# ultravideo/uvg266

Measured on AMD Instinct MI355X. Metric: encoded fps (1080p all-intra --preset medium closed loop: CTU search with the reference's RD decisions -> deblock -> SAO -> slice data; Mpixels/s in config), higher is better.
Workload: dtype u8

## Files before the change

### uvg266_amd/csrc/ctu_core.h

```cpp
#pragma once
#include <stdint.h>
#include <stddef.h>
#include <string.h>
#include "intra_pred_dev.h"
#if defined(__HIPCC__)
#include "satd_dev.h"
#endif
#include "vvc_tables.h"
#include "vvc_ctx_init.h"
#include "vvc_rdoq_tables.h"
#include "../../include/uvg266_hip.h"
#if defined(CTU_PB)
#include "inter_cand_dev.h"
#endif

#if defined(__HIPCC__)
#define CTU_NOINLINE __attribute__((noinline))
#define CTU_INLINE __attribute__((always_inline))
#define CTU_INLINE1 __attribute__((always_inline))
#define CTU_DEV static __device__
#define CTU_SHARED __shared__
#define CTU_TID ((int)(threadIdx.x & 63))
#define CTU_NT 64
#define CTU_WAVE (__builtin_amdgcn_readfirstlane((int)((threadIdx.x >> 6) - S->rot) & 3))
#define CTU_SYNC() do { __builtin_amdgcn_fence(__ATOMIC_ACQ_REL, "wavefront"); __builtin_amdgcn_wave_barrier(); } while (0)
#define BLK_TID ((int)threadIdx.x)
#define BLK_NT ((int)blockDim.x)
#define BLK_SYNC() __syncthreads()
#define CTU_GLOAD(p) __builtin_nontemporal_load(p)
#define CTU_LDS __attribute__((address_space(3)))
#define CTU_GLB __attribute__((address_space(1)))
#else
#define CTU_NOINLINE
#define CTU_INLINE
#define CTU_INLINE1
#define CTU_DEV static inline
#define CTU_SHARED static
#define CTU_TID 0
#define CTU_NT 1
#define CTU_WAVE (ctu::g_emul_wave)
#define CTU_SYNC() ((void)0)
#define BLK_TID 0
#define BLK_NT 1
#define BLK_SYNC() ((void)0)
#define CTU_GLOAD(p) (*(p))
#define CTU_LDS
#define CTU_GLB
#endif
#if defined(CTU_PB)
#define CTU_RQ_ROOT(V) ((V)->rq_root)
#else
#define CTU_RQ_ROOT(V) 0
#endif
#if defined(__HIPCC__) && defined(CTU_PROFILE)
#define CTU_T0() const unsigned long long ctu_t0__ = __builtin_amdgcn_s_memtime()
#define CTU_T1(W, slot) do { if (CTU_TID == 0) (W)->prof[CTU_WAVE][slot] += __builtin_amdgcn_s_memtime() - ctu_t0__; } while (0)
#define RQ_T0(W) scratch *const rq_w__ = (W); unsigned long long tq = __builtin_amdgcn_s_memtime();
#define RQ_T(slot) do { const unsigned long long t2 = __builtin_amdgcn_s_memtime(); if (CTU_TID == 0) rq_w__->prof[CTU_WAVE][slot] += t2 - tq; tq = t2; } while (0)
#define LF_T0() unsigned long long tq = __builtin_amdgcn_s_memtime()
#define LF_T(slot) do { const unsigned long long t2 = __builtin_amdgcn_s_memtime(); if (CTU_TID == 0 && CTU_WAVE == 0) J.W->prof_lf[slot] += t2 - tq; tq = t2; } while (0)
#define LF_TR() do { tq = __builtin_amdgcn_s_memtime(); } while (0)
#define LF_TN(slot) do { const unsigned long long t2 = __builtin_amdgcn_s_memtime(); if (CTU_TID == 0 && CTU_WAVE == 0) J.W->prof_lf[slot] += (1ull << 40) + (t2 - tq); tq = t2; } while (0)
#define WAIT_EVAL(S, L) do { LF_T0(); wait_eval(S, L); LF_T((L) <= 2 ? 14 : 15); } while (0)
#define CTU_PROF_RESET(S, J) BLK_FOR(i, 4 * 32) (J).W->prof[i >> 5][i & 31] = 0; BLK_FOR(i, 16) (J).W->prof_lf[i] = 0; (S)->prof_w = (J).W;
#define PB_T0() const unsigned long long pb_t0__ = __builtin_amdgcn_s_memtime()
#if defined(CTU_PROFILE_WALK)
#define PB_T1(W, slot) do { if (CTU_TID == 0 && ((slot) >= 14 || CTU_WAVE == 0)) (W)->prof_pb[slot] += __builtin_amdgcn_s_memtime() - pb_t0__; } while (0)
#else
#define PB_T1(W, slot) do { if (CTU_TID == 0) (W)->prof_pb[slot] += __builtin_amdgcn_s_memtime() - pb_t0__; } while (0)
#endif
#define PB_COUNT(W, slot) SERIAL (W)->prof_pb[slot] += 1;
#define PB_PROF_RESET(S, J) BLK_FOR(i, 24) (J).W->prof_pb[i] = 0; BLK_FOR(i, 4 * 32) (J).W->prof[i >> 5][i & 31] = 0; (S)->prof_w = (J).W;
#else
#define CTU_T0() ((void)0)
#define CTU_T1(W, slot) ((void)0)
#define RQ_T0(W)
#define RQ_T(slot) ((void)0)
#define LF_T0() ((void)0)
#define LF_T(slot) ((void)0)
#define LF_TR() ((void)0)
#define LF_TN(slot) ((void)0)
#define WAIT_EVAL(S, L) wait_eval(S, L)
#define CTU_PROF_RESET(S, J)
#define PB_T0() ((void)0)
#define PB_T1(W, slot) ((void)0)
#define PB_COUNT(W, slot)
#define PB_PROF_RESET(S, J)
#endif
#define LDSP(T, p) ((CTU_LDS T *)(p))
#define MGP(PX, T, p) ((typename ctu::mg_ptr<PX, T>::type)(p))
#define PAR_FOR(i, n) for (int i = CTU_TID; i < (n); i += CTU_NT)
#define BLK_FOR(i, n) for (int i = BLK_TID; i < (n); i += BLK_NT)
#define SERIAL if (CTU_TID == 0)

namespace ctu {

#if !defined(__HIPCC__)
static int g_emul_wave = 0;
static int g_emul_lazy = 0;
static int g_emul_depthwave = 0;
static int g_emul_leafwave = 0;
template <typename F> static inline void emul_on_wave(int w, F fn)
{
  const int me = g_emul_wave;
  g_emul_wave = w;
  fn();
  g_emul_wave = me;
}
#endif

enum { LCU = 64, LCU_C = 32, PY = 68, PC = 36, NMODELS = 257 };
#if defined(CTU_PB)
enum { NMX = NMODELS + 18 };
#else
enum { NMX = NMODELS };
#endif
enum { M_SIGGRP = 0, M_SIG = 4, M_PAR = 28, M_GT1 = 70, M_GT2 = 112, M_LASTX = 154, M_LASTY = 194, M_CBF_LUMA = 234, M_CBF_CB = 238,
       M_CBF_CR = 240, M_SPLIT = 244, M_MPM = 253, M_PLANAR = 254, M_CHROMA_PRED = 256 };
enum { CU_NOTSET = 0, CU_INTRA = 1, CU_INTER = 2 };
#define CTU_MAX_DOUBLE 1.7976931348623157e308

using params = uvghip_ctu_params_t;

struct cu4 {
  uint8_t type, log2, cbf, luma_edges, chroma_edges, log2_c;
  int8_t mode, mode_chroma;
};

struct level_state {
  double cost, split_cost, split_bits;
  int x, y;
  int child;
  int type, mode, cbf;
  int has_chroma;
  int pending;
  int evalp, known, can;
  uint32_t split_tree, mode_type_tree;
#if defined(CTU_PB)
  int32_t mot[8];
  uint8_t fl[8];
  int32_t cbf4[4];
#endif
};

#if !defined(__HIPCC__)
template <typename PX> struct lds_cfg { enum { slim = 0, slim_scan = 0 }; };
#elif defined(CTU_PB)
template <typename PX> struct lds_cfg { enum { slim = 0, slim_scan = 1 }; };
#else
template <typename PX> struct lds_cfg { enum { slim = 0, slim_scan = 0 }; };
template <> struct lds_cfg<uint16_t> { enum { slim = 1, slim_scan = 1 }; };
#endif
template <typename PX, typename T, bool SLIM = (lds_cfg<PX>::slim != 0)> struct mg_ptr { typedef CTU_LDS T *type; };
template <typename PX, typename T> struct mg_ptr<PX, T, true> { typedef T *type; };

template <typename PX> struct px_info;
template <> struct px_info<uint8_t> { enum { depth = 8, maxv = 255 }; };
template <> struct px_info<uint16_t> { enum { depth = 10, maxv = 1023 }; };

struct wctx {
// ... 158 lines not shown
template <typename PX> struct job {
  params P;
  const PX *src_y, *src_u, *src_v;
  int src_stride, src_stride_c;
  PX *rec_y, *rec_u, *rec_v;
  int rec_stride, rec_stride_c;
  uvghip_scu_t *cu_tab;
  int cu_stride;
  int16_t *coeff;
  uint32_t *models_out;
  const uint32_t *models_in;
  scratch *W;
  int x, y;
#if defined(CTU_PB)
  const struct pb_job *pb;
  uint32_t *pbm_out;
  const uint32_t *pbm_in;
  int slice_type, init_qp;
#endif
};

template <typename PX> CTU_DEV CTU_GLB const PX *src_block(const job<PX> &J, int color, int bx, int by, int *pitch)
{
  const PX *p = color == 0 ? J.src_y : (color == 1 ? J.src_u : J.src_v);
  const int st = color == 0 ? J.src_stride : J.src_stride_c, sh = color != 0;
  *pitch = st;
  return (CTU_GLB const PX *)(p + (size_t)((J.y >> sh) + by) * st + (J.x >> sh) + bx);
}


CTU_DEV uint32_t *tab_ebits() { CTU_SHARED uint32_t t[512]; return t; }
CTU_DEV uint8_t *tab_rate() { CTU_SHARED uint8_t t[(NMX + 7) & ~7]; return t; }
CTU_DEV uint32_t *tab_rdoq_bits() { CTU_SHARED uint32_t t[2 * 244]; return t; }
#define kRate (tab_rate())

template <typename MP> CTU_DEV int m_state(MP m, int c) { return (int)(((m[c] & 0xffffu) + (m[c] >> 16)) >> 8); }
template <typename MP> CTU_DEV void m_update(MP m, int c, int bin)
{
  const int r0 = kRate[c] >> 4, r1 = kRate[c] & 15;
  uint32_t s0 = m[c] & 0xffffu, s1 = m[c] >> 16;
  s0 -= (s0 >> r0) & 0x7fe0u;
  s1 -= (s1 >> r1) & 0x7ffeu;
  if (bin) { s0 += (0x7fffu >> r0) & 0x7fe0u; s1 += (0x7fffu >> r1) & 0x7ffeu; }
  m[c] = (s0 & 0xffffu) | (s1 << 16);
}
template <typename MP> CTU_DEV double m_fbits(MP m, int c, int bin) { return (double)tab_ebits()[(m_state(m, c) << 1) ^ bin] / 32768.0; }
template <typename MP> CTU_DEV void m_code(MP m, int update, int c, int bin, double &bits)
{
  bits += m_fbits(m, c, bin);
  if (update) m_update(m, c, bin);
}

CTU_DEV void models_init_one(uint32_t *m, int i, int qp, int slice)
{
  const int v = k_ctx_init[slice][i];
  if (v == 255) { m[i] = 0; return; }
  const int slope = (v >> 3) - 4, offset = ((v & 7) * 18) + 1;
  int s = ((slope * (qp - 16)) >> 1) + offset;
  s = s < 1 ? 1 : (s > 127 ? 127 : s);
  const uint32_t p1 = (uint32_t)s << 8;
  m[i] = (p1 & 0x7fe0u) | ((p1 & 0x7ffeu) << 16);
}

CTU_DEV int scan_base(int log2n) { return log2n == 5 ? 0 : log2n == 4 ? 1024 : log2n == 3 ? 1280 : 1344; }
template <typename PX> CTU_DEV uint16_t *scan_of(lds<PX> *S, int log2n)
{
  if (lds_cfg<PX>::slim_scan) return log2n >= 4 ? S->scr->scan_g + (log2n == 5 ? 0 : 1024) : S->scan + (log2n == 3 ? 0 : 64);
  return S->scan + scan_base(log2n);
}
CTU_DEV int last_bits_off(int t, int log2n, int xy)
{
  const int cnt = 2 * log2n;
  const int base = log2n == 2 ? 0 : (log2n == 3 ? 8 : (log2n == 4 ? 20 : 36));
  return (t ? 56 : 0) + base + (xy ? cnt : 0);
}
CTU_DEV void diag_order(int n, uint8_t *out)
{
  int i = 0;
  for (int d = 0; d < 2 * n - 1; ++d)
    for (int x = 0; x <= d; ++x) {
      const int y = d - x;
      if (x < n && y < n) out[i++] = (uint8_t)(y * n + x);
    }
}
template <typename PX> CTU_DEV void build_scans(lds<PX> *S)
{
  SERIAL {
    uint8_t in[16], cg[64];
    diag_order(4, in);
    for (int l2 = 2; l2 <= 5; ++l2) {
      const int n = 1 << l2, cgw = n >> 2;
      diag_order(cgw, cg);
      uint16_t *sc = scan_of(S, l2);
      if (l2 == 2) {
        for (int k = 0; k < 16; ++k) S->inv4[in[k]] = (uint8_t)k;
        for (int k = 0; k < 16; ++k) {
          const int x = in[k] & 3, y = in[k] >> 2;
          unsigned m = 0;
          if (x + 1 < 4) m |= 1u << S->inv4[y * 4 + x + 1];
          if (x + 2 < 4) m |= 1u << S->inv4[y * 4 + x + 2];
          if (y + 1 < 4) m |= 1u << S->inv4[(y + 1) * 4 + x];
          if (y + 2 < 4) m |= 1u << S->inv4[(y + 2) * 4 + x];
          if (x + 1 < 4 && y + 1 < 4) m |= 1u << S->inv4[(y + 1) * 4 + x + 1];
          S->deps4[k] = (uint16_t)m;
        }
      }
      for (int g = 0; g < cgw * cgw; ++g) {
        const int gx = cg[g] % cgw, gy = cg[g] / cgw;
        for (int k = 0; k < 16; ++k) sc[g * 16 + k] = (uint16_t)((gy * 4 + in[k] / 4) * n + gx * 4 + in[k] % 4);
      }
    }
  }
  CTU_SYNC();
}

CTU_DEV int16_t *lv_of(wctx *V, int color) { return color == 0 ? V->lv0 : (color == 1 ? V->lv1 : V->lv2); }
template <typename PX> CTU_DEV PX *plane(lds<PX> *S, int color) { return color == 0 ? S->Dy : (color == 1 ? S->Du : S->Dv); }
CTU_DEV int pitch_of(int color) { return color == 0 ? PY : PC; }
template <typename PX> CTU_DEV cu4 *cu_at(lds<PX> *S, int lx, int ly) { return &S->cu[((ly >> 2) + 1) * 17 + (lx >> 2) + 1]; }

template <typename PX> CTU_DEV int count_edge_cus(lds<PX> *S, int x, int y, int lx, int ly, int n, int left)
{
  if ((left && x == 0) || (!left && y == 0)) return 0;
  if (left && lx == 0) return (LCU - ly) / 4;
  if (!left && ly == 0) return n / 2;
  int amount = n & ~3;
  if (left) {
    if (ly == 0 && lx == 32 && cu_at(S, lx, ly)->log2 == 6) return 8;
    while (ly + amount < LCU && cu_at(S, lx - 4, ly + amount)->type != CU_NOTSET) amount += 4;
  } else {
    while (lx + amount < LCU && cu_at(S, lx + amount, ly - 4)->type != CU_NOTSET) amount += 4;
  }
  return (amount / 4) > (n / 4) ? amount / 4 : n / 4;
}

template <typename PX> CTU_NOINLINE CTU_DEV void build_refs(lds<PX> *S, const params &P, int color, int x, int y, int lx, int ly, int n, int cu_n)
{
  wctx *const V = wv_of(S);
  const int c = color != 0;
  const int w = n >> c;
  const int px_x = lx >> c, px_y = ly >> c;
  const int pit = pitch_of(color);
  const PX *D = plane(S, color) + (px_y + 1) * pit + px_x + 1;
  SERIAL {
    int al = count_edge_cus(S, x, y, lx, ly, n, 1) * (c ? 2 : 4);
    if (al > 2 * w) al = 2 * w;
    if (al > ((P.pic_h - y) >> c)) al = (P.pic_h - y) >> c;
    int at = count_edge_cus(S, x, y, lx, ly, n, 0) * (c ? 2 : 4);
    if (at > 2 * w) at = 2 * w;
    if (at > ((P.pic_w - x) >> c)) at = (P.pic_w - x) >> c;
    if (x > 0 && y > 0 && P.wpp && px_y == 0 && at > (LCU >> c) - px_x) at = (LCU >> c) - px_x;
    V->u_avail_left = al; V->u_avail_top = at;
  }
  CTU_SYNC();
  const int al = V->u_avail_left, at = V->u_avail_top;
  const int dc = 1 << (px_info<PX>::depth - 1);
  CTU_LDS uint16_t *const r_top = LDSP(uint16_t, V->top), *const r_left = LDSP(uint16_t, V->left);
  CTU_LDS uint16_t *const r_ftop = LDSP(uint16_t, V->ftop), *const r_fleft = LDSP(uint16_t, V->fleft);
  PAR_FOR(i, V->refn - 1) {
    int lv, tv;
    if (x > 0) lv = D[(i < al ? i : al - 1) * pit - 1];
    else lv = y > 0 ? D[-pit] : dc;
    if (y > 0) tv = D[-pit + (i < at ? i : at - 1)];
    else tv = x > 0 ? D[-1] : dc;
    r_left[i + 1] = (uint16_t)lv;
    r_top[i + 1] = (uint16_t)tv;
// ... 780 lines not shown
      const int o = off + (ctx >> sh);
      const int mx = M_LASTX + (E.t ? 20 : 0) + o, my = M_LASTY + (E.t ? 20 : 0) + o;
      last_x_bits[ctx] = bx + rbits(E, mx, 0); bx += rbits(E, mx, 1);
      last_y_bits[ctx] = by + rbits(E, my, 0); by += rbits(E, my, 1);
    }
    last_x_bits[ctx] = bx; last_y_bits[ctx] = by;
  }
  int found_last = 0;
  for (cgs = cg_last_scanpos; cgs >= 0; cgs--) {
    const int first = scan[cgs * 16];
    const int cg_blkpos = ((first >> l2) >> 2) * cgw + ((first & (n - 1)) >> 2);
    base_cost -= cost_cg_sig[cgs];
    if (cg_flag[cg_blkpos]) {
      for (int sp = 15; sp >= 0; sp--) {
        const int scanpos = cgs * 16 + sp;
        if (scanpos > last_scanpos) continue;
        const int blkpos = scan[scanpos];
        if (dst[blkpos]) {
          const int pos_y = blkpos >> l2, pos_x = blkpos - (pos_y << l2);
          const int cx = group_idx(pos_x), cy = group_idx(pos_y);
          double cl = last_x_bits[cx] + last_y_bits[cy];
          if (cx > 3) cl += 32768 * ((cx - 2) >> 1);
          if (cy > 3) cl += 32768 * ((cy - 2) >> 1);
          const double cost_last = lambda * cl;
          const double total = base_cost + cost_last - cost_sig[scanpos];
          if (total < best_cost) { best_last_idx_p1 = scanpos + 1; best_cost = total; }
          if (dst[blkpos] > 1) { found_last = 1; break; }
          base_cost -= cost_coeff[scanpos];
          base_cost += cost_coeff0[scanpos];
        } else {
          base_cost -= cost_sig[scanpos];
        }
      }
      if (found_last) break;
    }
  }
  int any = 0;
  for (int scanpos = 0; scanpos < best_last_idx_p1; scanpos++) {
    const int b = scan[scanpos], level = dst[b];
    any |= level;
    dst[b] = (int16_t)((coef[b] < 0) ? -level : level);
  }
  for (int scanpos = best_last_idx_p1; scanpos <= last_scanpos; scanpos++) dst[scan[scanpos]] = 0;
  return any != 0;
}

struct rdoq_pos { int level; double cc, cs; };
template <typename DP> CTU_INLINE CTU_DEV rdoq_pos rdoq_decide_inl(const rdoq_env &E, CTU_LDS const int16_t *coef, DP dst, int n, int l2, int color, int blkpos, bool is_last,
                             bool regular, int go_rice, double c0, int *mal_out)
{
  const int cap_half = 1 << (E.q_bits - 1);
  const int64_t prod = (int64_t)iabs_((int)coef[blkpos]) * E.q;
  const int32_t cap = 0x7fffffff - cap_half;
  const int32_t level_double = (int32_t)(prod < cap ? prod : cap);
  const uint32_t max_abs_level = (uint32_t)(level_double + cap_half) >> E.q_bits;
  const int pos_y = blkpos >> l2, pos_x = blkpos - (pos_y << l2);
  int ctx_sig = 0, ctx_set = 0;
  if (!is_last) {
    int diag, tsum;
    ctx_sig = sig_ctx_abs(dst, pos_x, pos_y, n, color, &diag, &tsum);
    ctx_set = ((tsum < 4 ? tsum : 4) + 1) + (!diag ? ((color == 0) ? 15 : 5) : (color == 0) ? (diag < 3 ? 10 : (diag < 10 ? 5 : 0)) : 0);
  }
  if (!regular) go_rice = go_rice_par(template_abs_sum(dst, 0, pos_x, pos_y, n));
  rdoq_pos r;
  r.cs = 0;
  r.level = (int)coded_level(E, &r.cc, c0, &r.cs, level_double, max_abs_level, ctx_sig, ctx_set, go_rice, regular ? 4u : 0u, is_last);
  *mal_out = (int)max_abs_level;
  return r;
}
template <typename DP> CTU_NOINLINE CTU_DEV rdoq_pos rdoq_decide(const rdoq_env &E, CTU_LDS const int16_t *coef, DP dst, int n, int l2, int color, int blkpos, bool is_last,
                             bool regular, int go_rice, double c0, int *mal_out)
{
  return rdoq_decide_inl(E, coef, dst, n, l2, color, blkpos, is_last, regular, go_rice, c0, mal_out);
}

#if !defined(__HIPCC__)
#include "ctu_rdoq_emul.h"
#else
CTU_DEV double rl64(double v, int lane)
{
  const int lo = __builtin_amdgcn_readlane(__double2loint(v), lane), hi = __builtin_amdgcn_readlane(__double2hiint(v), lane);
  return __hiloint2double(hi, lo);
}
template <typename PX> CTU_INLINE1 CTU_DEV void rdoq_wave(lds<PX> *S, scratch *W, const int16_t *coef_, int16_t *dst_, int n, int color, int cbf_u, int qp_scaled,
                                              double lambda, int bitdepth)
{
  wctx *const V = wv_of(S);
  CTU_LDS const int16_t *const coef = LDSP(const int16_t, coef_);
  typename mg_ptr<PX, int16_t>::type const dst = MGP(PX, int16_t, dst_);
  const int l2 = ilog2_dev(n), nn = n * n, cgw = n >> 2;
  const uint16_t *scan = scan_of(S, l2);
  rdoq_env E;
  E.st = S->rdoq_state; E.t = color ? 1 : 0; E.lambda = lambda;
  const int transform_shift = 15 - bitdepth - l2;
  E.q_bits = 14 + qp_scaled / 6 + transform_shift;
  E.q = kQuantScales[qp_scaled % 6];
  double scale = 32768;
  scale = transform_shift >= 0 ? scale / kPow2[2 * transform_shift] : scale * kPow2[-2 * transform_shift];
  E.error_scale = scale / E.q / E.q;
  const bool small = V->rq_cc != nullptr;
  CTU_LDS double *const CCl = LDSP(double, V->rq_cc), *const CSl = LDSP(double, V->rq_cs);
  const bool d1 = S->vsel[CTU_WAVE] == 3;
  double *const CCg = d1 ? W->cost_coeff : W->cost_coeff0, *const CSg = d1 ? W->cost_sig : W->cost_coeff0 + 512;
  double *cost_cg_sig = (double *)V->t1;
  const int cap_half = 1 << (E.q_bits - 1);
  const int32_t cap = 0x7fffffff - cap_half;
  RQ_T0(W)
  int my_last = -1;
  PAR_FOR(sp, nn) {
    const int blk = scan[sp];
    const int64_t prod = (int64_t)iabs_((int)coef[blk]) * E.q;
    const int32_t level_double = (int32_t)(prod < cap ? prod : cap);
    const int mal = (int)((uint32_t)(level_double + cap_half) >> E.q_bits);
    dst[blk] = (int16_t)mal;
    if (mal > 0 && sp > my_last) my_last = sp;
    if (sp < 64) V->cg_flag[sp] = 0;
  }
  for (int o = 32; o >= 1; o >>= 1) { const int v = __shfl_xor(my_last, o, 64); my_last = v > my_last ? v : my_last; }
  const int last_scanpos = my_last;
  CTU_SYNC();
  if (last_scanpos < 0) { if (CTU_TID == 0) V->rq_i[1] = 0; CTU_SYNC(); return; }
  RQ_T(12);
  const int cg_last = last_scanpos >> 4;
  const int lane = CTU_TID, sp = lane & 15;
  const bool own = lane < 16;
  double tail_cost = 0;
  {
    const auto tail_c0 = [&](int top) -> double {
      const int scanpos = top + sp;
      const int64_t prod = (int64_t)iabs_((int)coef[scan[scanpos]]) * E.q;
      const double err = (double)(int32_t)(prod < cap ? prod : cap);
      return scanpos > last_scanpos ? err * err * E.error_scale : 0.0;
    };
    double nxt = nn - 1 > last_scanpos ? tail_c0(nn - 16) : 0.0;
    for (int top = nn - 16; top + 15 > last_scanpos; top -= 16) {
      const double c0 = nxt;
      if (top - 1 > last_scanpos) nxt = tail_c0(top - 16);
#pragma unroll
      for (int k = 15; k >= 8; --k) tail_cost += rl64(c0, k);
      if (top + 7 > last_scanpos) {
#pragma unroll
        for (int k = 7; k >= 0; --k) tail_cost += rl64(c0, k);
      }
    }
  }
  double block_uncoded_cost = tail_cost, base_cost = tail_cost;
  if (CTU_TID == 0) for (int g = 0; g <= cg_last; ++g) cost_cg_sig[g] = 0;
  int reg_bins = (int)((uint32_t)(nn * 28) >> 4);
  CTU_SYNC();
  RQ_T(13);
  double f_cc = 0, f_cs = 0, f_c0 = 0;
  int f_lev = 0;
  for (int cgs = cg_last; cgs >= 0; --cgs) {
    const int first = scan[cgs * 16];
    const int cg_pos_x = (first & (n - 1)) >> 2, cg_pos_y = (first >> l2) >> 2;
    const int cg_blkpos = cg_pos_y * cgw + cg_pos_x;
    const int regular = reg_bins >= 4;
    const int scanpos = cgs * 16 + sp;
    const bool mine = own && scanpos <= last_scanpos;
    const int blk = scan[mine ? scanpos : cgs * 16];
    const bool is_last = scanpos == last_scanpos;
    const int64_t prod = (int64_t)iabs_((int)coef[blk]) * E.q;
    const int32_t level_double = (int32_t)(prod < cap ? prod : cap);
    const int mal0 = mine ? (int)((uint32_t)(level_double + cap_half) >> E.q_bits) : 0;
    const double c0 = mine ? (double)level_double * (double)level_double * E.error_scale : 0.0;
    int fast = !regular;
    if (regular) {
      int bound = mine ? (mal0 < 2 ? mal0 : 3) + (is_last ? 0 : 1) : 0;
      for (int o = 8; o >= 1; o >>= 1) bound += __shfl_xor(bound, o, 64);
      bound = __builtin_amdgcn_readfirstlane(bound);
      fast = reg_bins - bound >= 4;
    }
    double cc = 0, cs = 0;
    int lev = 0;
    if (fast) {
      int go_rice = 0;
      if (mine && regular && sp != 15 && !is_last) {
        const int nb = scan[scanpos + 1];
        go_rice = go_rice_par(template_abs_sum(coef, 4, nb & (n - 1), nb >> l2, n));
      }
      lev = mal0;
      for (;;) {
        bool changed = false;
        if (mine) {
          int mal;
          const rdoq_pos r = rdoq_decide_inl(E, coef, dst, n, l2, color, blk, is_last, regular != 0, go_rice, c0, &mal);
          cc = r.cc; cs = r.cs;
          changed = r.level != lev;
          lev = r.level;
        }
        CTU_SYNC();
        if (changed) dst[blk] = (int16_t)lev;
        const bool any = __ballot(changed) != 0;
        CTU_SYNC();
        if (!any) break;
      }
    } else {
      if (CTU_TID == 0) {
        int go_rice = 0, rb = reg_bins;
        for (int k = 15; k >= 0; --k) {
          const int spos = cgs * 16 + k;
          if (spos > last_scanpos) continue;
          const int b = scan[spos];
          const int64_t pr = (int64_t)iabs_((int)coef[b]) * E.q;
          const double e0 = (double)(int32_t)(pr < cap ? pr : cap);
          int mal;
          const rdoq_pos r = rdoq_decide(E, coef, dst, n, l2, color, b, spos == last_scanpos, rb >= 4, go_rice, e0 * e0 * E.error_scale, &mal);
          dst[b] = (int16_t)r.level;
          V->rq_stage[k] = r.cc; V->rq_stage[16 + k] = r.cs;
          if ((spos % 16 == 0) && spos > 0) go_rice = 0;
          else if (rb >= 4) {
            rb -= (r.level < 2 ? r.level : 3) + (spos != last_scanpos);
            go_rice = go_rice_par(template_abs_sum(coef, 4, b & (n - 1), b >> l2, n));
          }
        }
        V->rq_i[4] = rb;
      }
      CTU_SYNC();
      if (mine) { cc = V->rq_stage[sp]; cs = V->rq_stage[16 + sp]; lev = dst[blk]; }
      reg_bins = V->rq_i[4];
      CTU_SYNC();
    }
    RQ_T(14);
    double rd_coded = 0, rd_uncoded = 0, rd_sig = 0;
    const unsigned m_nz = (unsigned)__ballot(lev != 0), m_gt1 = (unsigned)__ballot(lev > 1), m_mine = (unsigned)__ballot(mine);
    const unsigned paying = cgs ? ~1u : ~0u, not_last = cgs == cg_last ? ~(1u << (last_scanpos & 15)) : ~0u;
    const int spent = __popc(m_nz & paying) + 2 * __popc(m_gt1 & paying) + __popc(m_mine & paying & not_last);
    const int nnz_before_pos0 = __popc(m_nz & ~1u);
    int flag = cgs && m_nz;
    const bool upper = cgs < cg_last || (last_scanpos & 15) >= 8;
    if (cgs) {
      const double dc = lev ? cc - cs : 0.0, du = lev ? c0 : 0.0;
      if (upper) {
#pragma unroll
        for (int k = 15; k >= 8; --k) {
          block_uncoded_cost += rl64(c0, k); base_cost += rl64(cc, k);
          rd_sig += rl64(cs, k); rd_coded += rl64(dc, k); rd_uncoded += rl64(du, k);
        }
      }
#pragma unroll
      for (int k = 7; k >= 0; --k) {
        block_uncoded_cost += rl64(c0, k); base_cost += rl64(cc, k);
        rd_sig += rl64(cs, k); rd_coded += rl64(dc, k); rd_uncoded += rl64(du, k);
      }
    } else {
      if (upper) {
#pragma unroll
        for (int k = 15; k >= 8; --k) { block_uncoded_cost += rl64(c0, k); base_cost += rl64(cc, k); }
      }
#pragma unroll
      for (int k = 7; k >= 0; --k) { block_uncoded_cost += rl64(c0, k); base_cost += rl64(cc, k); }
    }
    const double rd_sig0 = rl64(cs, 0);
    if (fast && regular) reg_bins -= spent;
    int zeroed = 0;
    if (cgs) {
      unsigned right = 0, lower = 0;
      if (cg_pos_x + 1 < cgw) right = V->cg_flag[cg_blkpos + 1];
      if (cg_pos_y + 1 < cgw) lower = V->cg_flag[cg_blkpos + cgw];
      const int o_grp = M_SIGGRP + (E.t ? 2 : 0) + ((right || lower) ? 1 : 0);
      double cgc = 0;
      if (!flag) {
        cgc = lambda * rbits(E, o_grp, 0);
        base_cost += cgc - rd_sig;
      } else if (cgs < cg_last) {
        if (nnz_before_pos0 == 0) { base_cost -= rd_sig0; rd_sig -= rd_sig0; }
        double cost_zero_cg = base_cost;
        cgc = lambda * rbits(E, o_grp, 1);
        base_cost += cgc;
        cost_zero_cg += lambda * rbits(E, o_grp, 0);
        cost_zero_cg += rd_uncoded;
        cost_zero_cg -= rd_coded;
        cost_zero_cg -= rd_sig;
        if (cost_zero_cg < base_cost) {
          flag = 0;
          zeroed = 1;
          base_cost = cost_zero_cg;
          cgc = lambda * rbits(E, o_grp, 0);
        }
      }
      CTU_SYNC();
      if (CTU_TID == 0) cost_cg_sig[cgs] = cgc;
    } else {
      flag = 1;
    }
    if (CTU_TID == 0) V->cg_flag[cg_blkpos] = (uint8_t)flag;
    if (cg_last == 0) { f_cc = cc; f_cs = cs; f_c0 = c0; f_lev = lev; }
    else if (mine) {
      const double wc = (zeroed && lev) ? c0 : cc, ws = (zeroed && lev) ? 0.0 : cs;
      if (zeroed && lev) dst[blk] = 0;
      if (small) { CCl[scanpos] = wc; CSl[scanpos] = ws; } else { CCg[scanpos] = wc; CSg[scanpos] = ws; }
    }
    CTU_SYNC();
    RQ_T(15);
  }
  RQ_T(16);
  double best_cost;
  int best_last_idx_p1 = 0;
  {
    const int o_cbf = color == 0 ? (CTU_RQ_ROOT(V) ? 243 : M_CBF_LUMA) : color == 1 ? M_CBF_CB : M_CBF_CR + (cbf_u ? 1 : 0);
    best_cost = block_uncoded_cost + lambda * rbits(E, o_cbf, 0);
    base_cost += lambda * rbits(E, o_cbf, 1);
  }
  const int32_t *last_x_bits = S->last_bits + last_bits_off(E.t, l2, 0), *last_y_bits = S->last_bits + last_bits_off(E.t, l2, 1);
  int found_last = 0;
  for (int cgs = cg_last; cgs >= 0 && !found_last; cgs--) {
    const int first = scan[cgs * 16];
    const int cg_blkpos = ((first >> l2) >> 2) * cgw + ((first & (n - 1)) >> 2);
    base_cost -= cost_cg_sig[cgs];
    if (!V->cg_flag[cg_blkpos]) continue;
    const int scanpos = cgs * 16 + sp;
    const bool mine = own && scanpos <= last_scanpos;
    const int blkpos = scan[mine ? scanpos : cgs * 16];
    const int lev = cg_last == 0 ? f_lev : (mine ? (int)dst[blkpos] : 0);
    double kcs = 0, kcc = 0, k0 = 0, klast = 0;
    if (mine) {
      kcs = cg_last == 0 ? f_cs : (small ? CSl[scanpos] : CTU_GLOAD(&CSg[scanpos]));
      if (lev) {
        if (cg_last == 0) { kcc = f_cc; k0 = f_c0; }
        else {
          kcc = small ? CCl[scanpos] : CTU_GLOAD(&CCg[scanpos]);
          const int64_t prod = (int64_t)iabs_((int)coef[blkpos]) * E.q;
          const double err = (double)(int32_t)(prod < cap ? prod : cap);
          k0 = err * err * E.error_scale;
        }
        const int pos_y = blkpos >> l2, pos_x = blkpos - (pos_y << l2);
        const int cx = group_idx(pos_x), cy = group_idx(pos_y);
        double cl = last_x_bits[cx] + last_y_bits[cy];
        if (cx > 3) cl += 32768 * ((cx - 2) >> 1);
        if (cy > 3) cl += 32768 * ((cy - 2) >> 1);
        klast = lambda * cl;
      }
    }
    const double kx = lev ? kcc : kcs;
    const unsigned m_nz = (unsigned)__ballot(lev != 0), m_gt1 = (unsigned)__ballot(lev > 1);
    const int kstop = m_gt1 ? 31 - __clz(m_gt1) : 0;
    const unsigned cand = m_nz >> kstop << kstop;
    if (cgs < cg_last || (last_scanpos & 15) >= 8) {
#pragma unroll
      for (int k = 15; k >= 8; --k) {
        const double total = base_cost + rl64(klast, k) - rl64(kcs, k);
        const bool better = (cand >> k & 1u) != 0 && total < best_cost;
        best_last_idx_p1 = better ? cgs * 16 + k + 1 : best_last_idx_p1;
        best_cost = better ? total : best_cost;
        base_cost = base_cost - rl64(kx, k) + rl64(k0, k);
      }
    }
    if (kstop < 8) {
#pragma unroll
      for (int k = 7; k >= 0; --k) {
        const double total = base_cost + rl64(klast, k) - rl64(kcs, k);
        const bool better = (cand >> k & 1u) != 0 && total < best_cost;
        best_last_idx_p1 = better ? cgs * 16 + k + 1 : best_last_idx_p1;
        best_cost = better ? total : best_cost;
        base_cost = base_cost - rl64(kx, k) + rl64(k0, k);
      }
    }
    found_last = m_gt1 != 0;
  }
  if (CTU_TID == 0) V->rq_i[1] = best_last_idx_p1 > 0;
  RQ_T(17);
  PAR_FOR(scanpos, last_scanpos + 1) {
    const int b = scan[scanpos];
    if (scanpos < best_last_idx_p1) { const int level = dst[b]; dst[b] = (int16_t)((coef[b] < 0) ? -level : level); }
    else dst[b] = 0;
  }
  CTU_SYNC();
  RQ_T(18);
}
#endif

CTU_DEV int coeff_remain_bits(uint32_t remainder, uint32_t rice, unsigned cutoff)
{
  const unsigned threshold = cutoff << rice;
  if (remainder < threshold) return (int)((remainder >> rice) + 1 + rice);
  const unsigned max_prefix = 32 - cutoff - 15;
  unsigned prefix = 0, suffix_len;
  const unsigned code_value = (remainder >> rice) - cutoff;
  if ((int32_t)code_value >= ((1 << max_prefix) - 1)) { prefix = max_prefix; suffix_len = 15; }
  else { while ((int32_t)code_value > ((2 << prefix) - 2)) prefix++; suffix_len = prefix + rice + 1; }
  return (int)(prefix + cutoff + suffix_len);
}
template <typename LP> CTU_DEV int abs_sum_tmpl(LP coeff, int px, int py, int n, int baselevel)
{
  const auto d = coeff + px + py * n;
  int sum = 0;
  if (px < n - 1) {
    sum += iabs_((int)d[1]);
    if (px < n - 2) sum += iabs_((int)d[2]);
    if (py < n - 1) sum += iabs_((int)d[n + 1]);
  }
  if (py < n - 1) {
    sum += iabs_((int)d[n]);
    if (py < n - 2) sum += iabs_((int)d[n << 1]);
  }
  int v = sum - 5 * baselevel;
  v = v < 31 ? v : 31;
  return v > 0 ? v : 0;
}

CTU_NOINLINE CTU_DEV double coeff_bits_serial(uint32_t *m, const uint16_t *scan, const int16_t *coeff, int n, int color)
{
  const int l2 = ilog2_dev(n);
  const int t = color ? 1 : 0;
  const int cgw = n >> 2;
  uint8_t sig_cg[64];
  for (int i = 0; i < cgw * cgw; ++i) sig_cg[i] = 0;
  int scan_pos_last = -1;
  for (int i = 0; i < n * n; ++i)
    if (coeff[scan[i]]) {
      scan_pos_last = i;
      const int f = scan[i & ~15];
      sig_cg[((f >> l2) >> 2) * cgw + ((f & (n - 1)) >> 2)] = 1;
    }
  if (scan_pos_last < 0) return 0;
  const int scan_cg_last = scan_pos_last >> 4;
  double bits_out = 0;
  {
// ... 1684 lines not shown
```

Before: 229.3.

## Batch RDOQ coefficient-group decisions across anti-diagonal using all 64 lanes

```diff
diff --git a/uvg266_amd/csrc/ctu_core.h b/uvg266_amd/csrc/ctu_core.h
--- a/uvg266_amd/csrc/ctu_core.h
+++ b/uvg266_amd/csrc/ctu_core.h
@@ -57,6 +57,7 @@
 #define CTU_T1(W, slot) do { if (CTU_TID == 0) (W)->prof[CTU_WAVE][slot] += __builtin_amdgcn_s_memtime() - ctu_t0__; } while (0)
 #define RQ_T0(W) scratch *const rq_w__ = (W); unsigned long long tq = __builtin_amdgcn_s_memtime();
 #define RQ_T(slot) do { const unsigned long long t2 = __builtin_amdgcn_s_memtime(); if (CTU_TID == 0) rq_w__->prof[CTU_WAVE][slot] += t2 - tq; tq = t2; } while (0)
+#define RQ_N(slot, v) if (CTU_TID == 0) rq_w__->prof[CTU_WAVE][slot] += (unsigned long long)(v) << 40;
 #define LF_T0() unsigned long long tq = __builtin_amdgcn_s_memtime()
 #define LF_T(slot) do { const unsigned long long t2 = __builtin_amdgcn_s_memtime(); if (CTU_TID == 0 && CTU_WAVE == 0) J.W->prof_lf[slot] += t2 - tq; tq = t2; } while (0)
 #define LF_TR() do { tq = __builtin_amdgcn_s_memtime(); } while (0)
@@ -76,6 +77,7 @@
 #define CTU_T1(W, slot) ((void)0)
 #define RQ_T0(W)
 #define RQ_T(slot) ((void)0)
+#define RQ_N(slot, v)
 #define LF_T0() ((void)0)
 #define LF_T(slot) ((void)0)
 #define LF_TR() ((void)0)
@@ -400,6 +402,10 @@
       const int y = d - x;
       if (x < n && y < n) out[i++] = (uint8_t)(y * n + x);
     }
+}
+CTU_DEV int rdoq_diag_start(int n, int d)
+{
+  return d < n ? d * (d + 1) / 2 : n * n - (2 * n - 1 - d) * (2 * n - d) / 2;
 }
 template <typename PX> CTU_DEV void build_scans(lds<PX> *S)
 {
@@ -1346,6 +1352,11 @@
   const int lo = __builtin_amdgcn_readlane(__double2loint(v), lane), hi = __builtin_amdgcn_readlane(__double2hiint(v), lane);
   return __hiloint2double(hi, lo);
 }
+CTU_DEV double shfl64(double v, int from)
+{
+  const int lo = __shfl(__double2loint(v), from, 64), hi = __shfl(__double2hiint(v), from, 64);
+  return __hiloint2double(hi, lo);
+}
 template <typename PX> CTU_INLINE1 CTU_DEV void rdoq_wave(lds<PX> *S, scratch *W, const int16_t *coef_, int16_t *dst_, int n, int color, int cbf_u, int qp_scaled,
                                               double lambda, int bitdepth)
 {
@@ -1413,149 +1424,172 @@
   int reg_bins = (int)((uint32_t)(nn * 28) >> 4);
   CTU_SYNC();
   RQ_T(13);
-  double f_cc = 0, f_cs = 0, f_c0 = 0;
-  int f_lev = 0;
-  for (int cgs = cg_last; cgs >= 0; --cgs) {
-    const int first = scan[cgs * 16];
-    const int cg_pos_x = (first & (n - 1)) >> 2, cg_pos_y = (first >> l2) >> 2;
-    const int cg_blkpos = cg_pos_y * cgw + cg_pos_x;
-    const int regular = reg_bins >= 4;
-    const int scanpos = cgs * 16 + sp;
-    const bool mine = own && scanpos <= last_scanpos;
-    const int blk = scan[mine ? scanpos : cgs * 16];
-    const bool is_last = scanpos == last_scanpos;
-    const int64_t prod = (int64_t)iabs_((int)coef[blk]) * E.q;
-    const int32_t level_double = (int32_t)(prod < cap ? prod : cap);
-    const int mal0 = mine ? (int)((uint32_t)(level_double + cap_half) >> E.q_bits) : 0;
-    const double c0 = mine ? (double)level_double * (double)level_double * E.error_scale : 0.0;
-    int fast = !regular;
-    if (regular) {
-      int bound = mine ? (mal0 < 2 ? mal0 : 3) + (is_last ? 0 : 1) : 0;
-      for (int o = 8; o >= 1; o >>= 1) bound += __shfl_xor(bound, o, 64);
-      bound = __builtin_amdgcn_readfirstlane(bound);
-      fast = reg_bins - bound >= 4;
-    }
-    double cc = 0, cs = 0;
-    int lev = 0;
-    if (fast) {
-      int go_rice = 0;
-      if (mine && regular && sp != 15 && !is_last) {
-        const int nb = scan[scanpos + 1];
-        go_rice = go_rice_par(template_abs_sum(coef, 4, nb & (n - 1), nb >> l2, n));
-      }
-      lev = mal0;
-      for (;;) {
-        bool changed = false;
-        if (mine) {
-          int mal;
-          const rdoq_pos r = rdoq_decide_inl(E, coef, dst, n, l2, color, blk, is_last, regular != 0, go_rice, c0, &mal);
-          cc = r.cc; cs = r.cs;
-          changed = r.level != lev;
-          lev = r.level;
+  const int row = lane >> 4;
+  double cc = 0, cs = 0, c0 = 0;
+  int lev = 0, ng = 0, r = 0, counted = 0;
+  for (int cgs = cg_last; cgs >= 0; --cgs, ++r) {
+    if (r == ng) {
+      const int top = cgs;
+      const int ftop = scan[top * 16];
+      const int dg = ((ftop & (n - 1)) >> 2) + ((ftop >> l2) >> 2);
+      const int dstart = rdoq_diag_start(cgw, dg);
+      ng = top - dstart + 1 < 4 ? top - dstart + 1 : 4;
+      r = 0;
+      const int regular = reg_bins >= 4;
+      const int cgr = row < ng ? top - row : top;
+      const int scanpos = cgr * 16 + sp;
+      const bool mine0 = row < ng && scanpos <= last_scanpos;
+      const int blk = scan[mine0 ? scanpos : cgr * 16];
+      const bool is_last = scanpos == last_scanpos;
+      const int64_t prod = (int64_t)iabs_((int)coef[blk]) * E.q;
+      const int32_t level_double = (int32_t)(prod < cap ? prod : cap);
+      const int mal1 = (int)((uint32_t)(level_double + cap_half) >> E.q_bits);
+      int fast = !regular;
+      if (regular) {
+        int bound = mine0 ? (mal1 < 2 ? mal1 : 3) + (is_last ? 0 : 1) : 0;
+        for (int o = 8; o >= 1; o >>= 1) bound += __shfl_xor(bound, o, 64);
+        const int b0 = __builtin_amdgcn_readlane(bound, 0);
+        const int all = b0 + __builtin_amdgcn_readlane(bound, 16) + __builtin_amdgcn_readlane(bound, 32) + __builtin_amdgcn_readlane(bound, 48);
+        fast = reg_bins - all >= 4;
+        if (!fast && ng > 1) { ng = 1; fast = reg_bins - b0 >= 4; RQ_N(13, 1) }
+      }
+      RQ_N(14, 1) RQ_N(15, ng)
+      const bool mine = mine0 && row < ng;
+      const int mal0 = mine ? mal1 : 0;
+      c0 = mine ? (double)level_double * (double)level_double * E.error_scale : 0.0;
+      cc = 0; cs = 0;
+      lev = 0;
+      counted = fast && regular;
+      if (fast) {
+        int go_rice = 0;
+        if (mine && regular && sp != 15 && !is_last) {
+          const int nb = scan[scanpos + 1];
+          go_rice = go_rice_par(template_abs_sum(coef, 4, nb & (n - 1), nb >> l2, n));
+        }
+        lev = mal0;
+        for (;;) {
+          bool changed = false;
+          RQ_N(12, 1)
+          if (mine) {
+            int mal;
+            const rdoq_pos r = rdoq_decide_inl(E, coef, dst, n, l2, color, blk, is_last, regular != 0, go_rice, c0, &mal);
+            cc = r.cc; cs = r.cs;
+            changed = r.level != lev;
+            lev = r.level;
+          }
+          CTU_SYNC();
+          if (changed) dst[blk] = (int16_t)lev;
+          const bool any = __ballot(changed) != 0;
+          CTU_SYNC();
+          if (!any) break;
+        }
+      } else {
+        if (CTU_TID == 0) {
+          int go_rice = 0, rb = reg_bins;
+          for (int k = 15; k >= 0; --k) {
+            const int spos = top * 16 + k;
+            if (spos > last_scanpos) continue;
+            const int b = scan[spos];
+            const int64_t pr = (int64_t)iabs_((int)coef[b]) * E.q;
+            const double e0 = (double)(int32_t)(pr < cap ? pr : cap);
+            int mal;
+            const rdoq_pos r = rdoq_decide(E, coef, dst, n, l2, color, b, spos == last_scanpos, rb >= 4, go_rice, e0 * e0 * E.error_scale, &mal);
+            dst[b] = (int16_t)r.level;
+            V->rq_stage[k] = r.cc; V->rq_stage[16 + k] = r.cs;
+            if ((spos % 16 == 0) && spos > 0) go_rice = 0;
+            else if (rb >= 4) {
+              rb -= (r.level < 2 ? r.level : 3) + (spos != last_scanpos);
+              go_rice = go_rice_par(template_abs_sum(coef, 4, b & (n - 1), b >> l2, n));
+            }
+          }
+          V->rq_i[4] = rb;
         }
         CTU_SYNC();
-        if (changed) dst[blk] = (int16_t)lev;
-        const bool any = __ballot(changed) != 0;
+        if (mine) { cc = V->rq_stage[sp]; cs = V->rq_stage[16 + sp]; lev = dst[blk]; }
+        reg_bins = V->rq_i[4];
         CTU_SYNC();
-        if (!any) break;
-      }
+      }
+      RQ_T(14);
     } else {
-      if (CTU_TID == 0) {
-        int go_rice = 0, rb = reg_bins;
-        for (int k = 15; k >= 0; --k) {
-          const int spos = cgs * 16 + k;
-          if (spos > last_scanpos) continue;
-          const int b = scan[spos];
-          const int64_t pr = (int64_t)iabs_((int)coef[b]) * E.q;
-          const double e0 = (double)(int32_t)(pr < cap ? pr : cap);
-          int mal;
-          const rdoq_pos r = rdoq_decide(E, coef, dst, n, l2, color, b, spos == last_scanpos, rb >= 4, go_rice, e0 * e0 * E.error_scale, &mal);
-          dst[b] = (int16_t)r.level;
-          V->rq_stage[k] = r.cc; V->rq_stage[16 + k] = r.cs;
-          if ((spos % 16 == 0) && spos > 0) go_rice = 0;
-          else if (rb >= 4) {
-            rb -= (r.level < 2 ? r.level : 3) + (spos != last_scanpos);
-            go_rice = go_rice_par(template_abs_sum(coef, 4, b & (n - 1), b >> l2, n));
+      const int from = (lane + 16) & 63;
+      cc = shfl64(cc, from); cs = shfl64(cs, from); c0 = shfl64(c0, from); lev = __shfl(lev, from, 64);
+    }
+    {
+      const int first = scan[cgs * 16];
+      const int cg_pos_x = (first & (n - 1)) >> 2, cg_pos_y = (first >> l2) >> 2;
+      const int cg_blkpos = cg_pos_y * cgw + cg_pos_x;
+      const int gpos = cgs * 16 + sp;
+      const bool gmine = own && gpos <= last_scanpos;
+      double rd_coded = 0, rd_uncoded = 0, rd_sig = 0;
+      const unsigned m_nz = (unsigned)__ballot(lev != 0) & 0xffffu, m_gt1 = (unsigned)__ballot(lev > 1) & 0xffffu, m_mine = (unsigned)__ballot(gmine);
+      const unsigned paying = cgs ? ~1u : ~0u, not_last = cgs == cg_last ? ~(1u << (last_scanpos & 15)) : ~0u;
+      const int spent = __popc(m_nz & paying) + 2 * __popc(m_gt1 & paying) + __popc(m_mine & paying & not_last);
+      const int nnz_before_pos0 = __popc(m_nz & ~1u);
+      int flag = cgs && m_nz;
+      const bool upper = cgs < cg_last || (last_scanpos & 15) >= 8;
+      if (cgs) {
+        const double dc = lev ? cc - cs : 0.0, du = lev ? c0 : 0.0;
+        if (upper) {
+#pragma unroll
+          for (int k = 15; k >= 8; --k) {
+            block_uncoded_cost += rl64(c0, k); base_cost += rl64(cc, k);
+            rd_sig += rl64(cs, k); rd_coded += rl64(dc, k); rd_uncoded += rl64(du, k);
           }
         }
-        V->rq_i[4] = rb;
-      }
-      CTU_SYNC();
-      if (mine) { cc = V->rq_stage[sp]; cs = V->rq_stage[16 + sp]; lev = dst[blk]; }
-      reg_bins = V->rq_i[4];
-      CTU_SYNC();
-    }
-    RQ_T(14);
-    double rd_coded = 0, rd_uncoded = 0, rd_sig = 0;
-    const unsigned m_nz = (unsigned)__ballot(lev != 0), m_gt1 = (unsigned)__ballot(lev > 1), m_mine = (unsigned)__ballot(mine);
-    const unsigned paying = cgs ? ~1u : ~0u, not_last = cgs == cg_last ? ~(1u << (last_scanpos & 15)) : ~0u;
-    const int spent = __popc(m_nz & paying) + 2 * __popc(m_gt1 & paying) + __popc(m_mine & paying & not_last);
-    const int nnz_before_pos0 = __popc(m_nz & ~1u);
-    int flag = cgs && m_nz;
-    const bool upper = cgs < cg_last || (last_scanpos & 15) >= 8;
-    if (cgs) {
-      const double dc = lev ? cc - cs : 0.0, du = lev ? c0 : 0.0;
-      if (upper) {
 #pragma unroll
-        for (int k = 15; k >= 8; --k) {
+        for (int k = 7; k >= 0; --k) {
           block_uncoded_cost += rl64(c0, k); base_cost += rl64(cc, k);
           rd_sig += rl64(cs, k); rd_coded += rl64(dc, k); rd_uncoded += rl64(du, k);
         }
-      }
+      } else {
+        if (upper) {
 #pragma unroll
-      for (int k = 7; k >= 0; --k) {
-        block_uncoded_cost += rl64(c0, k); base_cost += rl64(cc, k);
-        rd_sig += rl64(cs, k); rd_coded += rl64(dc, k); rd_uncoded += rl64(du, k);
-      }
-    } else {
-      if (upper) {
+          for (int k = 15; k >= 8; --k) { block_uncoded_cost += rl64(c0, k); base_cost += rl64(cc, k); }
+        }
 #pragma unroll
-        for (int k = 15; k >= 8; --k) { block_uncoded_cost += rl64(c0, k); base_cost += rl64(cc, k); }
-      }
-#pragma unroll
-      for (int k = 7; k >= 0; --k) { block_uncoded_cost += rl64(c0, k); base_cost += rl64(cc, k); }
-    }
-    const double rd_sig0 = rl64(cs, 0);
-    if (fast && regular) reg_bins -= spent;
-    int zeroed = 0;
-    if (cgs) {
-      unsigned right = 0, lower = 0;
-      if (cg_pos_x + 1 < cgw) right = V->cg_flag[cg_blkpos + 1];
-      if (cg_pos_y + 1 < cgw) lower = V->cg_flag[cg_blkpos + cgw];
-      const int o_grp = M_SIGGRP + (E.t ? 2 : 0) + ((right || lower) ? 1 : 0);
-      double cgc = 0;
-      if (!flag) {
-        cgc = lambda * rbits(E, o_grp, 0);
-        base_cost += cgc - rd_sig;
-      } else if (cgs < cg_last) {
-        if (nnz_before_pos0 == 0) { base_cost -= rd_sig0; rd_sig -= rd_sig0; }
-        double cost_zero_cg = base_cost;
-        cgc = lambda * rbits(E, o_grp, 1);
-        base_cost += cgc;
-        cost_zero_cg += lambda * rbits(E, o_grp, 0);
-        cost_zero_cg += rd_uncoded;
-        cost_zero_cg -= rd_coded;
-        cost_zero_cg -= rd_sig;
-        if (cost_zero_cg < base_cost) {
-          flag = 0;
-          zeroed = 1;
-          base_cost = cost_zero_cg;
+        for (int k = 7; k >= 0; --k) { block_uncoded_cost += rl64(c0, k); base_cost += rl64(cc, k); }
+      }
+      const double rd_sig0 = rl64(cs, 0);
+      if (counted) reg_bins -= spent;
+      int zeroed = 0;
+      if (cgs) {
+        unsigned right = 0, lower = 0;
+        if (cg_pos_x + 1 < cgw) right = V->cg_flag[cg_blkpos + 1];
+        if (cg_pos_y + 1 < cgw) lower = V->cg_flag[cg_blkpos + cgw];
+        const int o_grp = M_SIGGRP + (E.t ? 2 : 0) + ((right || lower) ? 1 : 0);
+        double cgc = 0;
+        if (!flag) {
           cgc = lambda * rbits(E, o_grp, 0);
+          base_cost += cgc - rd_sig;
+        } else if (cgs < cg_last) {
+          if (nnz_before_pos0 == 0) { base_cost -= rd_sig0; rd_sig -= rd_sig0; }
+          double cost_zero_cg = base_cost;
+          cgc = lambda * rbits(E, o_grp, 1);
+          base_cost += cgc;
+          cost_zero_cg += lambda * rbits(E, o_grp, 0);
+          cost_zero_cg += rd_uncoded;
+          cost_zero_cg -= rd_coded;
+          cost_zero_cg -= rd_sig;
+          if (cost_zero_cg < base_cost) {
+            flag = 0;
+            zeroed = 1;
+            base_cost = cost_zero_cg;
+            cgc = lambda * rbits(E, o_grp, 0);
+          }
         }
+        CTU_SYNC();
+        if (CTU_TID == 0) cost_cg_sig[cgs] = cgc;
+      } else {
+        flag = 1;
+      }
+      if (CTU_TID == 0) V->cg_flag[cg_blkpos] = (uint8_t)flag;
+      if (cg_last != 0 && gmine) {
+        const double wc = (zeroed && lev) ? c0 : cc, ws = (zeroed && lev) ? 0.0 : cs;
+        if (zeroed && lev) dst[scan[gpos]] = 0;
+        if (small) { CCl[gpos] = wc; CSl[gpos] = ws; } else { CCg[gpos] = wc; CSg[gpos] = ws; }
       }
       CTU_SYNC();
-      if (CTU_TID == 0) cost_cg_sig[cgs] = cgc;
-    } else {
-      flag = 1;
-    }
-    if (CTU_TID == 0) V->cg_flag[cg_blkpos] = (uint8_t)flag;
-    if (cg_last == 0) { f_cc = cc; f_cs = cs; f_c0 = c0; f_lev = lev; }
-    else if (mine) {
-      const double wc = (zeroed && lev) ? c0 : cc, ws = (zeroed && lev) ? 0.0 : cs;
-      if (zeroed && lev) dst[blk] = 0;
-      if (small) { CCl[scanpos] = wc; CSl[scanpos] = ws; } else { CCg[scanpos] = wc; CSg[scanpos] = ws; }
-    }
-    CTU_SYNC();
+    }
     RQ_T(15);
   }
   RQ_T(16);
@@ -1576,12 +1610,12 @@
     const int scanpos = cgs * 16 + sp;
     const bool mine = own && scanpos <= last_scanpos;
     const int blkpos = scan[mine ? scanpos : cgs * 16];
-    const int lev = cg_last == 0 ? f_lev : (mine ? (int)dst[blkpos] : 0);
+    const int klev = cg_last == 0 ? lev : (mine ? (int)dst[blkpos] : 0);
     double kcs = 0, kcc = 0, k0 = 0, klast = 0;
     if (mine) {
-      kcs = cg_last == 0 ? f_cs : (small ? CSl[scanpos] : CTU_GLOAD(&CSg[scanpos]));
-      if (lev) {
-        if (cg_last == 0) { kcc = f_cc; k0 = f_c0; }
+      kcs = cg_last == 0 ? cs : (small ? CSl[scanpos] : CTU_GLOAD(&CSg[scanpos]));
+      if (klev) {
+        if (cg_last == 0) { kcc = cc; k0 = c0; }
         else {
           kcc = small ? CCl[scanpos] : CTU_GLOAD(&CCg[scanpos]);
           const int64_t prod = (int64_t)iabs_((int)coef[blkpos]) * E.q;
@@ -1596,8 +1630,8 @@
         klast = lambda * cl;
       }
     }
-    const double kx = lev ? kcc : kcs;
-    const unsigned m_nz = (unsigned)__ballot(lev != 0), m_gt1 = (unsigned)__ballot(lev > 1);
+    const double kx = klev ? kcc : kcs;
+    const unsigned m_nz = (unsigned)__ballot(klev != 0), m_gt1 = (unsigned)__ballot(klev > 1);
     const int kstop = m_gt1 ? 31 - __clz(m_gt1) : 0;
     const unsigned cand = m_nz >> kstop << kstop;
     if (cgs < cg_last || (last_scanpos & 15) >= 8) {
```

Result: faster. 233.9, median of 6 (+2.0%).
